# xyzy/jubatus

Measured on AMD Instinct MI355X. Metric: train_samples_per_sec, higher is better.
Workload: dtype fp32

## Files before the change

jubatus_amd/csrc/hip/jb_vc_state.hpp:

```cpp
#pragma once
#include <stdint.h>

#include "jb_serial_layout.hpp"

namespace jb {
namespace vc {

enum : int { kNew = 0, kRetry = 1, kDone = 2, kDense = 3 };
enum : int {
  S_MAGIC = 0, S_BEG, S_BEND, S_STATUS, S_LW, S_T, S_NCAND, S_PEND, S_WHY, S_NUPD, S_NSLOTS, S_VIOL,
  S_DONEB, S_NVALID, S_RETRYW, S_WEND,
  S_WINDOWS, S_RETRIES, S_STEPS, S_ROUNDS, S_WASTED, S_REFRESH, S_EXACT, S_CAND, S_UPD, S_SAT, S_TICKS,
  S_NONC, S_PH0, S_PH1, S_PH2, S_PH3, S_PH4, S_PHW, S_WIDE, S_DENSE_PM,
  S_DCHUNK,
  S_STEPPED,
  S_NCHUNK,
  S_BBEG,
  S_CSMODE,
  S_CSN,
  S_NWORDS = 64
};
enum : int { kWhyEnd = 0, kWhySat = 1, kWhyDense = 2 };
constexpr int64_t kDenseChunk0 = 8192, kDenseChunkMax = 1 << 20;

constexpr int kSpSlotBytes = 98304;
__host__ __device__ constexpr int sp_nslot(int lc) {
  return kSpSlotBytes / (8 * lc) > 1024 ? 1024 : kSpSlotBytes / (8 * lc);
}
__device__ __forceinline__ void sp_buckets(int row, int nb, int* b1, int* b2) {
  const uint32_t h1 = (uint32_t)row * 0x9E3779B1u;
  uint32_t h2 = ((uint32_t)row ^ 0x5bd1e995u) * 0x85EBCA77u;
  h2 ^= h2 >> 13;
  h2 *= 0xC2B2AE35u;
  *b1 = (int)__umulhi(h1, (uint32_t)nb);
  int c = (int)__umulhi(h2, (uint32_t)nb);
  if (c == *b1) c = c + 1 == nb ? 0 : c + 1;
  *b2 = c;
}
__device__ __forceinline__ int sp_find(const int32_t* key, int nb, int32_t row) {
  if (row < 0) return -1;
  int b1, b2;
  sp_buckets(row, nb, &b1, &b2);
  const int4 k1 = reinterpret_cast<const int4*>(key)[b1];
  const int4 k2 = reinterpret_cast<const int4*>(key)[b2];
  int s = -1;
  s = k1.x == row ? 4 * b1 : s;
  s = k1.y == row ? 4 * b1 + 1 : s;
  s = k1.z == row ? 4 * b1 + 2 : s;
  s = k1.w == row ? 4 * b1 + 3 : s;
  s = k2.x == row ? 4 * b2 : s;
  s = k2.y == row ? 4 * b2 + 1 : s;
  s = k2.z == row ? 4 * b2 + 2 : s;
  s = k2.w == row ? 4 * b2 + 3 : s;
  return s;
}

__device__ inline int64_t seg_estimate(const int64_t* st) {
  const int64_t wins = st[S_WINDOWS], stepped = st[S_STEPPED];
  const int64_t committed = st[S_BEG] - st[S_BBEG] - stepped;
  int64_t per = committed > 0 && wins > 0 ? committed / wins : 2048;
  per = per < 1024 ? 1024 : per;
  return wins + st[S_RETRIES] + (stepped + per - 1) / per;
}

}
}
```

jubatus_amd/csrc/hip/serial.hip:

```cpp
#include "jb_linear.hpp"
#include "jb_serial_layout.hpp"
#include <cstdio>
#include <cstdlib>
#include <algorithm>
#include <mutex>
#include <unordered_map>

namespace jb {

constexpr int kCommitThreads = 512;
constexpr int kDBits = 14;
constexpr int kDCap = 1 << kDBits;
constexpr int kDProbe = 32;
constexpr int kDFull = kDCap * 5 / 8;
constexpr int kBloomBits = 16;
constexpr int kSerialNF = 16;
constexpr float kSlackGuard = 1e-4f;
constexpr int kStepBits = 8;
constexpr int kStepCap = 1 << kStepBits;
constexpr int kStepList = 64;
constexpr int kSerialSegments = 4;
constexpr int kSerialSegmentsBig = 48;
constexpr int64_t kSerialBigBatch = 16384;
constexpr int kVerifiedSegmentsMin = 8;
constexpr int kVerifiedSegmentsMax = 2048;
constexpr int kRescoreWaste = 16;
constexpr int kScoreMaxBlocks = 8192;
#ifndef JB_SERIAL_TIMING
#define JB_SERIAL_TIMING 0
#endif
constexpr bool kSerialTiming = JB_SERIAL_TIMING != 0;
__device__ __forceinline__ uint64_t stamp() { return kSerialTiming ? clock64() : 0; }

template <int LC>
__device__ __forceinline__ void sample_scores_ro(const int32_t* __restrict__ fidx,
                                                 const float* __restrict__ fval, int64_t beg, int n,
                                                 const float* __restrict__ W, int lane,
                                                 float (&acc)[Lanes<LC>::K]) {
  using L = Lanes<LC>;
  const int g = lane / L::LW;
  const int l0 = lane % L::LW;
#pragma unroll
  for (int k = 0; k < L::K; ++k) acc[k] = 0.f;
  for (int j = g; j < n; j += L::G) {
    const int32_t idx = fidx[beg + j];
    const float x = fval[beg + j];
    if (idx >= 0) {
      const float* wr = W + (int64_t)idx * LC + l0;
#pragma unroll
      for (int k = 0; k < L::K; ++k) acc[k] += x * wr[64 * k];
    }
  }
#pragma unroll
  for (int off = L::LW; off < 64; off <<= 1) {
#pragma unroll
    for (int k = 0; k < L::K; ++k) acc[k] += __shfl_xor(acc[k], off, 64);
  }
}

template <int LC>
__device__ __forceinline__ float margin_of(const float (&acc)[Lanes<LC>::K], int y,
                                           const bool (&act)[Lanes<LC>::K], int lane, int* lstar,
                                           float* sy_out, float* best_out) {
  using L = Lanes<LC>;
  const int l0 = lane % L::LW;
  float sy = 0.f, best = -INFINITY;
  int bl = -1;
#pragma unroll
  for (int k = 0; k < L::K; ++k) {
    const int l = l0 + 64 * k;
    if (l == y) sy = acc[k];
    if (act[k] && l != y && acc[k] > best) { best = acc[k]; bl = l; }
  }
  sy = __shfl(sy, y % L::LW, 64);
  argmax_wrong<L::LW>(best, bl);
  *lstar = bl;
  *sy_out = sy;
  *best_out = bl >= 0 ? best : 0.f;
  return sy - (bl >= 0 ? best : 0.f);
}

__device__ __forceinline__ float decision_slack(int method, float margin, float nrm, bool has_l,
                                                float C, float sy, float best) {
  float s;
// ... 493 lines not shown
      if (k == INT_MAX) break;
      if (tid == k) {
        if (!loaded) load_features<NF>(fi, fx, live, nf, fb, fidx, fval);
        s_n = nf;
        s_y = yl;
        s_fb = fb;
        if (nf <= NF)
          for (int u = 0; u < nf; ++u) { s_fi[u] = fi[u]; s_fx[u] = fx[u]; }
      }
      if (wv == 0) {
        d.step_clear(lane);
        __builtin_amdgcn_wave_barrier();
        if (lane == 0) s_sn = 0;
      }
      lds_barrier();
      { const uint64_t t = stamp(); ph[2] += t - tc; tc = t; }
      if (wv == 0) {
        asm volatile("s_waitcnt vmcnt(0)" ::: "memory");
        const int n = s_n;
        bool up;
        if (kStaged && n <= NF)
          up = commit_staged<(LC <= 32 ? LC : 32)>(s_fi, s_fx, n, s_y, W, P, act[0], lane, method, C,
                                                   touched, d);
        else
          up = commit_sample<LC>(fidx, fval, s_fb, n, s_y, W, P, act, lane, method, C, touched, d);
        if (up) ++n_upd; else ++n_waste;
        if (lane == 0) s_waste = n_waste;
      }
      lim = k;
      ++steps;
      ++n_steps;
      { const uint64_t t = stamp(); ph[3] += t - tc; tc = t; }
      lds_barrier();
      { const uint64_t t = stamp(); ph[4] += t - tc; tc = t; }
      tw = stamp();
      if (s_sat || steps > bail_after || (rescore_waste > 0 && s_waste > rescore_waste)) {
        stop = p + k + 1;
        why = s_sat ? kStopSaturated : steps > bail_after ? kStopDense : kStopRescore;
        break;
      }
      if (loaded && open && tid > k && sl >= 0.f) {
        if (s_sn > kStepList || nf > NF) {
          bnd = full_bound();
        } else {
          bnd += d.step_bound<NF>(fi, fx);
        }
      }
    }
    ++n_rounds;
    const bool counted = live && !(sl != sl) && j < stop;
    const uint64_t cm = __builtin_amdgcn_ballot_w64(counted);
    if (lane == 0 && cm != 0) atomicAdd(&s_valid, (unsigned)__popcll(cm));
    if (stop != end) break;
  }
  __syncthreads();
  auto put = [&](int i, int64_t v) { tail[i] = seg == 0 ? v : tail[i] + v; };
  if (lane == 0) put(kTailBoundWave0 + wv, (int64_t)wwork);
  if (tid == 0) {
    tail[kTailStart] = stop;
    tail[kTailEnd] = end;
    tail[kTailReason] = why;
    put(kTailSteps, n_steps);
    put(kTailRounds, n_rounds);
    put(kTailSegments, 1);
    for (int i = 0; i < 6; ++i) put(kTailBoundPhase0 + i, (int64_t)ph[i]);
    put(kTailBoundWall, kSerialTiming ? (int64_t)(wall_clock64() - w0) : 0);
    put(kTailBoundCycles,
        (int64_t)(stamp() - tc) + (int64_t)(ph[0] + ph[1] + ph[2] + ph[3] + ph[4] + ph[5]));
    if (stats != nullptr && s_valid > 0) atomicAdd(stats + 1, (unsigned long long)s_valid);
  }
  if (tid == 0 && stats != nullptr && n_upd > 0) atomicAdd(stats, (unsigned long long)n_upd);
}

}

extern "C" int64_t jb_serial_scratch_bytes(int64_t n_max) {
  return jb::VcScratch::bytes(n_max > 0 ? n_max : 1);
}

extern "C" int64_t jb_serial_scratch_bytes_lc(int64_t n_max, int LC) {
  return LC > 64 ? jb::BoundScratch::bytes(n_max > 0 ? n_max : 1) : jb_serial_scratch_bytes(n_max);
}

enum : int { kSeenReason = 0, kSeenSegments, kSeenSegEst, kSeenWords };
static_assert(jb::kTailSegments == jb::kTailReason + 1, "one copy reads back both");
static std::mutex& seen_mu() {
  static std::mutex mu;
  return mu;
}
static std::unordered_map<void*, int64_t*>& seen_map() {
  static std::unordered_map<void*, int64_t*> seen;
  return seen;
}
static int64_t* segments_seen(void* scratch) {
  std::lock_guard<std::mutex> g(seen_mu());
  auto& seen = seen_map();
  auto it = seen.find(scratch);
  if (it != seen.end()) return it->second;
  int64_t* p = nullptr;
  if (hipHostMalloc((void**)&p, kSeenWords * sizeof(int64_t), hipHostMallocDefault) != hipSuccess) return nullptr;
  p[kSeenReason] = jb::kStopDone;
  p[kSeenSegments] = 128;
  p[kSeenSegEst] = 0;
  seen[scratch] = p;
  return p;
}

extern "C" int jb_vcommit_prepare(const int64_t* row_ptr, const int32_t* fidx, const float* fval,
                                  const int32_t* labels, const int64_t* stream_ptr, int nstreams, int64_t n_max,
                                  float* W, float* S, const int32_t* active, int LC, int method, float C,
                                  unsigned long long* stats, uint8_t* touched, void* scratch, int nseg,
                                  hipStream_t stream);

extern "C" int jb_serial_scratch_forget(void* scratch) {
  std::lock_guard<std::mutex> g(seen_mu());
  auto& seen = seen_map();
  auto it = seen.find(scratch);
  if (it == seen.end()) return 0;
  (void)hipHostFree(it->second);
  seen.erase(it);
  return 1;
}

static int segment_budget(int64_t n_max, int64_t prev, int64_t est, int64_t why) {
  if (n_max < jb::kSerialBigBatch) return jb::kVerifiedSegmentsMin;
  if (why != jb::kStopDone && why != jb::kStopDense) return jb::kVerifiedSegmentsMax;
  static const std::pair<int, int> slack = [] {
    const char* e = getenv("JB_VC_SEG_SLACK");
    int d = 2, c = 8;
    if (e != nullptr && sscanf(e, "%d,%d", &d, &c) != 2) { d = 2; c = 8; }
    return std::make_pair(d > 0 ? d : 2, c >= 0 ? c : 8);
  }();
  prev = std::max(prev, est);
  return (int)std::min<int64_t>(jb::kVerifiedSegmentsMax,
                                std::max<int64_t>(jb::kVerifiedSegmentsMin,
                                                  prev + prev / slack.first + slack.second));
}

extern "C" int jb_serial_prepare(const int64_t* row_ptr, const int32_t* fidx, const float* fval,
                                 const int32_t* labels, const int64_t* stream_ptr, int nstreams,
                                 int64_t n_max, float* W, float* S, const int32_t* active, int LC,
                                 int method, float C, unsigned long long* stats, uint8_t* touched,
                                 void* scratch, int64_t scratch_bytes, int bail_after,
                                 hipStream_t stream) {
  if (nstreams <= 0 || n_max <= 0) return 0;
  if (scratch == nullptr || scratch_bytes < jb_serial_scratch_bytes_lc(n_max, LC)) return -3;
  if (method >= jb::CW && S == nullptr) return -4;
  int64_t* tail = (int64_t*)scratch;
  if (LC <= 64) {
    volatile int64_t* seen = segments_seen(scratch);
    const int nseg = seen != nullptr
                         ? segment_budget(n_max, seen[kSeenSegments], seen[kSeenSegEst], seen[kSeenReason])
                         : segment_budget(n_max, 0, 0, jb::kStopDone);
    const int rc = jb_vcommit_prepare(row_ptr, fidx, fval, labels, stream_ptr, nstreams, n_max, W, S, active,
                                      LC, method, C, stats, touched, scratch, nseg, stream);
    if (rc == 0 && seen != nullptr) {
      int64_t* host = const_cast<int64_t*>(seen);
      (void)hipMemcpyAsync(host + kSeenReason, tail + jb::kTailReason, 2 * sizeof(int64_t), hipMemcpyDeviceToHost,
                           stream);
      (void)hipMemcpyAsync(host + kSeenSegEst, tail + jb::kTailSegEst, sizeof(int64_t), hipMemcpyDeviceToHost,
                           stream);
    }
    return rc;
  }
  float* slack = (float*)((uint8_t*)scratch + jb::BoundScratch::slack_offset());
  float* l1n = (float*)((uint8_t*)scratch + jb::BoundScratch::l1_offset(n_max));
  const int64_t blocks = std::min<int64_t>((n_max * 64 + 255) / 256, jb::kScoreMaxBlocks);
  const int nseg = n_max >= jb::kSerialBigBatch ? jb::kSerialSegmentsBig : jb::kSerialSegments;
  static_assert(jb::kTailStart == 0 && jb::kTailEnd == 1, "the tail doubles as a one-stream stream_ptr");
  for (int seg = 0; seg < nseg; ++seg) {
    const int waste = seg + 1 < nseg ? jb::kRescoreWaste : 0;
    const int64_t* sp = seg == 0 ? stream_ptr : tail;
    const int ns = seg == 0 ? nstreams : 1;
    const int64_t* why = seg == 0 ? nullptr : tail + jb::kTailReason;
#define JB_SERIAL(L)                                                                              \
  hipLaunchKernelGGL((jb::serial_score_kernel<L>), dim3((unsigned)blocks), dim3(256), 0, stream,  \
                     row_ptr, fidx, fval, labels, sp, ns, W, active, method, C, slack, l1n, why); \
  hipLaunchKernelGGL((jb::serial_commit_kernel<L>), dim3(1), dim3(jb::kCommitThreads), 0, stream, \
                     row_ptr, fidx, fval, labels, sp, ns, W, S, active, method, C, slack, l1n,    \
                     stats, touched, tail, bail_after, seg, waste);                               \
  break;
    switch (LC) {
      case 128: JB_SERIAL(128)
      case 256: JB_SERIAL(256)
      case 512: JB_SERIAL(512)
      case 1024: JB_SERIAL(1024)
      default: return -1;
    }
#undef JB_SERIAL
  }
  return (int)hipGetLastError();
}
```

jubatus_amd/csrc/hip/vcommit.hip:

```cpp
#include <string.h>

#include <type_traits>

#include "jb_commit.hpp"
#include "jb_vc_state.hpp"

namespace jb {
namespace vc {

using dc::Geo;
constexpr int kFCMax = 2;
constexpr int kRec = 16 * kFCMax;
constexpr int64_t kLwMin = 2048, kLwMax = kVcWindowMax, kLwInit = 8192;
constexpr int kBitWords = kVcBitWords;
constexpr float kTInit = 0.5f, kTMin = 0.125f, kTMax = 64.f;
constexpr int64_t kMagic = 0x56434f4d4d495433LL;
constexpr int kRetryForce = 3;

__device__ __forceinline__ float st_T(const int64_t* st) { return __int_as_float((int)st[S_T]); }
__device__ __forceinline__ int64_t ld_st(const int64_t* p) {
  return __hip_atomic_load(p, __ATOMIC_RELAXED, __HIP_MEMORY_SCOPE_AGENT);
}
__device__ __forceinline__ bool live(int status) { return status == kNew || status == kRetry; }

__device__ __forceinline__ float frcp(float x) { return __builtin_amdgcn_rcpf(x); }
__device__ __forceinline__ bool step_coeffs_fast(int method, float margin, float var, float nrm, bool has_l, float C,
                                                 float* tau, float* beta) {
  switch (method) {
    case PERCEPTRON:
      if (margin <= 0.f) { *tau = 1.f; *beta = 0.f; return true; }
      return false;
    case PA: case PA1: case PA2: {
      const float loss = 1.f - margin;
      if (!(loss > 0.f && nrm > 0.f)) return false;
      const float sq = (has_l ? 2.f : 1.f) * nrm;
      if (method == PA) *tau = loss * frcp(sq);
      else if (method == PA1) *tau = fminf(C, loss * frcp(sq));
      else *tau = loss * frcp(sq + 0.5f * frcp(C));
      *beta = 0.f;
      return true;
    }
    case CW: {
      if (!(var > 0.f)) return false;
      const float phi = C;
      const float b = 1.f + 2.f * phi * margin;
      const float disc = b * b - 8.f * phi * (margin - phi * var);
      const float gamma = (-b + sqrtf(fmaxf(disc, 0.f))) * frcp(4.f * phi * var);
      if (!(gamma > 0.f)) return false;
      *tau = gamma; *beta = 2.f * gamma * phi;
      return true;
    }
    case AROW:
      if (!(margin < 1.f)) return false;
      *beta = frcp(var + frcp(C));
      *tau = (1.f - margin) * *beta;
      return true;
    case NHERD: {
      if (!(margin < 1.f)) return false;
      *tau = (1.f - margin) * frcp(var + frcp(C));
      const float cv = 1.f + C * var;
      *beta = (C * C * var + 2.f * C) * frcp(cv * cv);
      return true;
    }
    default: return false;
  }
}
__device__ __forceinline__ float dprec_fast(int method, float beta, float x, float s) {
  const float bx2 = beta * x * x;
  return method == CW ? bx2 : bx2 * frcp(1.f - bx2 * s);
}

__global__ __launch_bounds__(256) void vc_init_kernel(int64_t* __restrict__ st, const int64_t* __restrict__ sp,
                                                      int nstreams, unsigned long long* __restrict__ bits,
                                                      int64_t* __restrict__ tail, float t_force,
                                                      int32_t* __restrict__ g_key, float* __restrict__ g_rmax,
                                                      int dense_pm) {
  for (int i = threadIdx.x; i < kBitWords; i += blockDim.x) bits[i] = 0ull;
  const bool fresh = st[S_MAGIC] != kMagic;
  if (fresh)
    for (int i = threadIdx.x; i < 1024; i += blockDim.x) { g_key[i] = -1; g_rmax[i] = 0.f; }
  __syncthreads();
  if (threadIdx.x != 0) return;
  if (fresh) {
    for (int i = 0; i < S_NWORDS; ++i) st[i] = 0;
    st[S_MAGIC] = kMagic;
    st[S_LW] = kLwInit;
    st[S_T] = __float_as_int(kTInit);
  }
  if (t_force > 0.f) st[S_T] = __float_as_int(t_force);
  const int64_t beg = sp[0], bend = sp[nstreams];
  st[S_BEG] = beg;
  st[S_BEND] = bend;
  st[S_WEND] = beg;
  st[S_STATUS] = beg < bend ? kNew : kDone;
  for (int i = S_NCAND; i <= S_RETRYW; ++i) st[i] = 0;
  for (int i = S_WINDOWS; i < S_NWORDS; ++i) st[i] = 0;
  st[S_DENSE_PM] = dense_pm;
  st[S_DCHUNK] = kDenseChunk0;
  st[S_BBEG] = beg;
  for (int i = 0; i < kTailWords; ++i) tail[i] = 0;
  tail[kTailStart] = beg < bend ? beg : bend;
  tail[kTailEnd] = bend;
  tail[kTailVerified] = 1;
}

// ... 136 lines not shown
  const int g = lane / L::LW;
  const int l0 = lane % L::LW;
  const bool la = l0 < LC && active[l0] != 0;
  for (int64_t k = ((int64_t)blockIdx.x * blockDim.x + tid) >> 6; k < ncand; k += nwaves) {
    int lo = 0, hi = nw - 1;
    while (lo < hi) {
      const int mid = (lo + hi + 1) >> 1;
      if (s_pref[mid] <= k) lo = mid; else hi = mid - 1;
    }
    unsigned long long word = bits[lo];
    for (int j = (int)k - s_pref[lo]; j > 0; --j) word &= word - 1;
    const int pos = 64 * lo + (__ffsll((long long)word) - 1);
    const int64_t s = beg + pos;
    int n;
    float acc, q;
    wave_score<LC>(row_ptr, fidx, fval, W, s, lane, la, &n, &acc, &q);
    const int64_t fb = row_ptr[s];
    if (lane < kRec) {
      const bool in = lane < n;
      FI[k * kRec + lane] = in ? fidx[fb + lane] : -1;
      FX[k * kRec + lane] = in ? fval[fb + lane] : 0.f;
    }
    if (lane == 0 && n > 16) atomicOr((unsigned long long*)&st[S_WIDE], 1ull);
    if (lane < LC) S0[k * LC + lane] = acc;
    (void)g;
    const int y = labels[s];
    if (y < 0 || y >= LC) {
      if (lane == 0) AUX[k] = make_int4(dc::aux_pack(-1, -1, n), __float_as_int(q), __float_as_int(1.f), pos);
      continue;
    }
    int bl;
    const float sl0 = wave_slack<LC>(acc, y, la, lane, method, C, q, &bl);
    if (lane == 0) AUX[k] = make_int4(dc::aux_pack(y, bl, n), __float_as_int(q), __float_as_int(sl0), pos);
    if (P == nullptr) continue;
    if (lane < kRec) {
      float2 pp = make_float2(1.f, 1.f);
      if (lane < n) {
        const int32_t idx = fidx[fb + lane];
        if (idx >= 0) {
          pp.x = P[(int64_t)idx * LC + y];
          if (bl >= 0) pp.y = P[(int64_t)idx * LC + bl];
        }
      }
      PP0[k * kRec + lane] = pp;
    }
  }
}

template <int LC, int FC>
struct Raw {
  int32_t fi[FC];
  float fx[FC];
  float2 pp[FC];
  float s[Geo<LC>::K];
  int aux;
  float nrm;
  float slack0;
  int pos;
};

template <int LC, int FC>
struct Samp {
  int32_t fi[FC];
  float fx[FC];
  float py[FC];
  float pl[FC];
  float s[Geo<LC>::K];
  int y;
  int ls0;
  int nf;
  float nrm;
  float slack0;
  int pos;
};

struct __attribute__((aligned(16))) Stamp { float sid, dy, dl, rmax; };

template <int LC, int MT, int R_, int PD_, int FC_>
__global__ __launch_bounds__(64) void vc_commit_kernel(
    int64_t* __restrict__ st, const float* __restrict__ W, const float* __restrict__ P,
    const int32_t* __restrict__ active, float C, const float* __restrict__ S0_k,
    const int4* __restrict__ AUX_k, const float2* __restrict__ PP0_k, const int32_t* __restrict__ FI_k,
    const float* __restrict__ FX_k, int32_t* __restrict__ g_key, float* __restrict__ g_rmax,
    float* __restrict__ g_dw, float* __restrict__ g_dp, int prof) {
  using Gm = Geo<LC>;
  using Rw = Raw<LC, FC_>;
  using S = Samp<LC, FC_>;
  constexpr int kFC = FC_;
  constexpr int kNFM = 16 * FC_;
  constexpr int kR = R_;
  constexpr int kNS = 4 * R_;
  constexpr int kPD = PD_;
  constexpr int K = Gm::K;
  constexpr int NSLOT = Gm::NSLOT;
  constexpr int method = MT;
  constexpr bool use_s = MT >= CW;
  constexpr bool use_nrm = MT == PA || MT == PA1 || MT == PA2 || MT == CW;
  constexpr float kG = dc::kGuard;
  if (!live((int)st[S_STATUS])) return;
  if (st[S_CSMODE] == 1) return;
  if ((st[S_WIDE] != 0) != (FC_ == 2)) return;
  __shared__ __attribute__((aligned(16))) float s_dw[NSLOT * LC + Gm::PAD];
  __shared__ __attribute__((aligned(16))) float s_dp[use_s ? NSLOT * LC + Gm::PAD : 4];
  __shared__ __attribute__((aligned(16))) int32_t s_key[NSLOT];
  __shared__ __attribute__((aligned(16))) Stamp s_sg[NSLOT + 1];

  const int lane = threadIdx.x;
  const int sub = lane & 15;
  const int G = lane >> 4;
  const uint64_t t_k0 = __builtin_amdgcn_s_memrealtime();
  const uint64_t t_c0 = __builtin_amdgcn_s_memtime();
  {
    float4* dw4 = reinterpret_cast<float4*>(s_dw);
    float4* dp4 = reinterpret_cast<float4*>(s_dp);
    const float4 z = make_float4(0.f, 0.f, 0.f, 0.f);
    for (int i = lane; i < (NSLOT * LC + Gm::PAD) / 4; i += 64) {
      dw4[i] = z;
      if (use_s) dp4[i] = z;
    }
    for (int i = lane; i < NSLOT; i += 64) s_key[i] = -1;
    for (int i = lane; i <= NSLOT; i += 64) s_sg[i] = Stamp{__int_as_float(-1), 0.f, 0.f, 0.f};
  }
  int act[K];
#pragma unroll
  for (int k = 0; k < K; ++k) {
    const int lab = sub + 16 * k;
    act[k] = (lab < LC && active[lab] != 0) ? 1 : 0;
  }
  const int64_t ncand = (int64_t)dc::in_vgpr((uint64_t)st[S_NCAND]);
  const int64_t wb = (int64_t)dc::in_vgpr((uint64_t)st[S_BEG]);
  const int64_t we = (int64_t)dc::in_vgpr((uint64_t)st[S_WEND]);
  const float* __restrict__ S0 = dc::in_vgpr(S0_k);
  const int4* __restrict__ AUX = dc::in_vgpr(AUX_k);
  const float2* __restrict__ PP0 = dc::in_vgpr(PP0_k);
  const int32_t* __restrict__ FI = dc::in_vgpr(FI_k);
  const float* __restrict__ FX = dc::in_vgpr(FX_k);

  auto load_raw = [&](int64_t k0, Rw (&rw)[kR]) {
#pragma unroll
    for (int r = 0; r < kR; ++r) {
      int64_t j = k0 + G * kR + r;
      j = j < ncand ? j : ncand - 1;
      j = j < 0 ? 0 : j;
#pragma unroll
      for (int c = 0; c < kFC; ++c) {
        const int64_t o = j * kRec + c * 16 + sub;
        rw[r].fi[c] = dc::gld(FI + o);
        rw[r].fx[c] = dc::gld(FX + o);
        if (use_s) rw[r].pp[c] = dc::gld(PP0 + o);
      }
#pragma unroll
      for (int k = 0; k < K; ++k) {
        const int lab = sub + 16 * k;
        rw[r].s[k] = dc::gld(S0 + j * LC + (lab < LC ? lab : LC - 1));
      }
      const int* a = reinterpret_cast<const int*>(AUX + j);
      rw[r].aux = dc::gld(a);
      rw[r].slack0 = __int_as_float(dc::gld(a + 2));
      rw[r].pos = dc::gld(a + 3);
      if (use_nrm) rw[r].nrm = __int_as_float(dc::gld(a + 1));
    }
  };
  auto unpack = [&](int64_t k0, const Rw (&rw)[kR], S (&sm)[kR]) {
#pragma unroll
    for (int r = 0; r < kR; ++r) {
      const bool ok = k0 + G * kR + r < ncand;
#pragma unroll
      for (int c = 0; c < kFC; ++c) {
        sm[r].fi[c] = ok ? rw[r].fi[c] : -1;
        sm[r].fx[c] = ok ? rw[r].fx[c] : 0.f;
        sm[r].py[c] = (use_s && ok) ? rw[r].pp[c].x : 1.f;
        sm[r].pl[c] = (use_s && ok) ? rw[r].pp[c].y : 1.f;
      }
#pragma unroll
      for (int k = 0; k < K; ++k) sm[r].s[k] = (ok && sub + 16 * k < LC) ? rw[r].s[k] : 0.f;
      const int aux = rw[r].aux;
      sm[r].y = ok ? dc::aux_y(aux) : -1;
      sm[r].ls0 = (use_s && ok) ? dc::aux_ls(aux) : -1;
      sm[r].nf = ok ? dc::aux_nf(aux) : 0;
      sm[r].nrm = (use_nrm && ok) ? rw[r].nrm : 0.f;
      sm[r].slack0 = ok ? rw[r].slack0 : 1.f;
      sm[r].pos = rw[r].pos;
    }
  };
// ... 270 lines not shown
            cy = row16_sum(cy);
            cl = row16_sum(cl);
            if (exact[r]) {
#pragma unroll
              for (int kk = 0; kk < K; ++kk) {
                const int lab = sub + 16 * kk;
                if (lab == yk) sc[r].s[kk] += cy;
                if (lab == lk) sc[r].s[kk] += cl;
              }
            }
            slack[r] -= (fabsf(cy) + fabsf(cl)) * (1.f + 4.f * kG);
            if (exact[r] && !(slack[r] > 0.f)) {
              int ls2;
              float sy2, best2;
              const float m2 = dc::group_margin<LC>(sc[r].s, sc[r].y, act, sub, &ls2, &sy2, &best2);
              slack[r] = dc::slack_of(method, m2, sc[r].nrm, ls2 >= 0, C, sy2, best2);
            }
          }
          make_exact(k);
#pragma unroll
          for (int r = 0; r < kR; ++r)
            if (G * kR + r > k) unsafe[r] = (alive[r] && (sc[r].nf > kNFM || !(slack[r] > 0.f))) ? 1 : 0;
        }
        return 0;
      };
      int stop_code = 0;
      switch (rk) {
        case 0: stop_code = step_of(std::integral_constant<int, 0>{}); break;
        case 1: if constexpr (kR > 1) stop_code = step_of(std::integral_constant<int, (kR > 1 ? 1 : 0)>{}); break;
        case 2: if constexpr (kR > 2) stop_code = step_of(std::integral_constant<int, (kR > 2 ? 2 : 0)>{}); break;
        default: if constexpr (kR > 3) stop_code = step_of(std::integral_constant<int, (kR > 3 ? 3 : 0)>{}); break;
      }
      stamp(4);
      if (stop_code) break;
      lim = k;
    }
    bump(3);
  };
  for (int64_t p0 = 0; p0 < ncand && !stopped; p0 += kPD * kNS) {
#pragma unroll
    for (int u = 0; u < kPD; ++u) {
      const int64_t p = p0 + u * kNS;
      unpack(p, pf[u], sc);
      load_raw(p + kPD * kNS, pf[u]);
      if (p < ncand && !stopped) round(p);
    }
  }
  int nslots = 0;
  for (int i = lane; i < NSLOT; i += 64) {
    const int32_t key = s_key[i];
    g_key[i] = key;
    g_rmax[i] = s_sg[i].rmax;
    nslots += key >= 0;
  }
  {
    constexpr int Q = LC / 4;
    for (int i = lane; i < NSLOT * Q; i += 64) {
      if (s_key[i / Q] < 0) continue;
      reinterpret_cast<float4*>(g_dw)[i] = reinterpret_cast<const float4*>(s_dw)[i];
      if (use_s) reinterpret_cast<float4*>(g_dp)[i] = reinterpret_cast<const float4*>(s_dp)[i];
    }
  }
#pragma unroll
  for (int off = 1; off < 64; off <<= 1) nslots += __shfl_xor(nslots, off, 64);
  if (lane == 0) {
    st[S_PEND] = pend;
    st[S_WHY] = why;
    st[S_NUPD] = s_cnt[0];
    st[S_NSLOTS] = nslots;
    st[S_STEPS] += n_steps;
    st[S_ROUNDS] += s_cnt[3];
    st[S_WASTED] += s_cnt[1];
    st[S_REFRESH] += s_cnt[2];
    st[S_EXACT] += n_exact;
    st[S_CAND] += ncand;
    st[S_TICKS] += (int64_t)(__builtin_amdgcn_s_memrealtime() - t_k0);
    if (kProf) {
      for (int i = 0; i < 5; ++i) st[S_PH0 + i] += (int64_t)s_ph[i];
      st[S_PHW] += (int64_t)(__builtin_amdgcn_s_memtime() - t_c0);
    }
  }
}

template <int LC>
__global__ __launch_bounds__(256) void vc_verify_kernel(
    int64_t* __restrict__ st, const int64_t* __restrict__ row_ptr, const int32_t* __restrict__ fidx,
    const float* __restrict__ fval, const int32_t* __restrict__ labels, const float* __restrict__ SL,
    unsigned long long* __restrict__ bits, const int32_t* __restrict__ g_key,
    const float* __restrict__ g_rmax, const float* __restrict__ g_dw, const float* __restrict__ g_dp,
    float* __restrict__ W, float* __restrict__ P, uint8_t* __restrict__ touched,
    unsigned long long* __restrict__ stats, int64_t* __restrict__ tail) {
  using Gm = Geo<LC>;
  constexpr int NSLOT = Gm::NSLOT;
  constexpr float kG = dc::kGuard;
  const int status = (int)st[S_STATUS];
  if (!live(status)) return;
  __shared__ __attribute__((aligned(16))) int32_t s_key[NSLOT];
  __shared__ float s_rmax[NSLOT];
  __shared__ unsigned s_valid, s_viol;
  __shared__ int s_last, s_force;
  const int tid = threadIdx.x;
  for (int i = tid; i < NSLOT; i += blockDim.x) {
    s_key[i] = g_key[i];
    s_rmax[i] = g_rmax[i];
  }
  if (tid == 0) { s_valid = 0; s_viol = 0; }
  __syncthreads();
  const int64_t wb = st[S_BEG], pe = st[S_PEND];
  const bool cs_mode = st[S_CSMODE] == 1;
  unsigned nvalid = 0, nviol = 0, nnonc = 0;
  for (int64_t i = wb + (int64_t)blockIdx.x * blockDim.x + tid; i < pe; i += (int64_t)gridDim.x * blockDim.x) {
    const int y = labels[i];
    if (y < 0 || y >= LC) continue;
    ++nvalid;
    const int64_t rel = i - wb;
    const unsigned long long bit = 1ull << (rel & 63);
    if (bits[rel >> 6] & bit) continue;
    ++nnonc;
    float bound = 0.f;
    for (int64_t j = row_ptr[i]; j < row_ptr[i + 1]; ++j) {
      const int32_t row = fidx[j];
      if (row < 0) continue;
      const int s = cs_mode ? sp_find(s_key, sp_nslot(LC) / 4, row) : dc::cache_find<LC>(s_key, row);
      if (s >= 0) bound += fabsf(fval[j]) * s_rmax[s];
    }
    bound *= 2.f * (1.f + 4.f * kG);
    if (!(SL[rel] > bound)) {
      atomicOr(bits + (rel >> 6), bit);
      ++nviol;
    }
  }
  if (nvalid) atomicAdd(&s_valid, nvalid);
  if (nviol) atomicAdd(&s_viol, nviol);
  if (nnonc) atomicAdd((unsigned long long*)&st[S_NONC], (unsigned long long)nnonc);
  __syncthreads();
  if (tid == 0) {
    if (s_valid) atomicAdd((unsigned long long*)&st[S_NVALID], (unsigned long long)s_valid);
    if (s_viol) atomicAdd((unsigned long long*)&st[S_VIOL], (unsigned long long)s_viol);
    __threadfence();
    s_last = atomicAdd((unsigned long long*)&st[S_DONEB], 1ull) == (unsigned long long)(gridDim.x - 1);
  }
  __syncthreads();
  if (!s_last) return;
  __threadfence();
  const int64_t viol = ld_st(&st[S_VIOL]);
  const int64_t wend = st[S_WEND];
  if (viol == 0) {
    __shared__ int s_used[NSLOT];
    __shared__ int s_nused;
    if (tid == 0) s_nused = 0;
    __syncthreads();
    for (int i = tid; i < NSLOT; i += blockDim.x)
      if (s_key[i] >= 0) s_used[atomicAdd(&s_nused, 1)] = i;
    __syncthreads();
    constexpr int Q = LC / 4;
    constexpr int kU = 4;
    const int items = s_nused * Q;
    for (int b0 = 0; b0 < items; b0 += kU * (int)blockDim.x) {
      float4 w[kU], d[kU], pv[kU], dp[kU];
      int64_t off[kU];
      bool on[kU];
#pragma unroll
      for (int u = 0; u < kU; ++u) {
        const int it = b0 + u * (int)blockDim.x + tid;
        on[u] = it < items;
        const int sl = s_used[on[u] ? it / Q : 0];
        const int q = it % Q;
        off[u] = (int64_t)s_key[sl] * Q + q;
        const int gi = sl * Q + q;
        if (on[u]) {
          w[u] = reinterpret_cast<const float4*>(W)[off[u]];
          d[u] = reinterpret_cast<const float4*>(g_dw)[gi];
          if (P != nullptr) {
            pv[u] = reinterpret_cast<const float4*>(P)[off[u]];
            dp[u] = reinterpret_cast<const float4*>(g_dp)[gi];
          }
        }
      }
#pragma unroll
      for (int u = 0; u < kU; ++u) {
        if (!on[u]) continue;
        w[u].x += d[u].x; w[u].y += d[u].y; w[u].z += d[u].z; w[u].w += d[u].w;
        reinterpret_cast<float4*>(W)[off[u]] = w[u];
        if (P != nullptr) {
          pv[u].x += dp[u].x; pv[u].y += dp[u].y; pv[u].z += dp[u].z; pv[u].w += dp[u].w;
          reinterpret_cast<float4*>(P)[off[u]] = pv[u];
        }
        if (off[u] % Q == 0 && touched != nullptr) touched[off[u] / Q] = 1;
      }
    }
    for (int i = tid; i < kBitWords; i += blockDim.x) bits[i] = 0ull;
    if (tid == 0) {
      const int64_t nupd = st[S_NUPD];
      const int64_t nv = ld_st(&st[S_NVALID]);
      if (stats != nullptr) {
        if (nupd > 0) atomicAdd(stats, (unsigned long long)nupd);
        if (nv > 0) atomicAdd(stats + 1, (unsigned long long)nv);
      }
      const int why = (int)st[S_WHY];
      const int64_t bend = st[S_BEND];
      st[S_BEG] = pe;
      st[S_WINDOWS] += 1;
      st[S_UPD] += nupd;
      if (why == kWhySat) st[S_SAT] += 1;
      const int64_t dpm = st[S_DENSE_PM];
      const bool dense = dpm > 0 && pe < bend && nupd * 1000 > dpm * (pe - wb);
      st[S_STATUS] = (why == kWhyDense || dense) ? kDense : (pe >= bend ? kDone : kNew);
      if (!(why == kWhyDense || dense)) st[S_DCHUNK] = kDenseChunk0;
      int64_t lw = st[S_LW];
      if (why == kWhySat) {
        const int64_t took = pe - wb;
        lw = took + took / 4;
      } else if (pe - wb >= lw) {
        lw = 2 * lw;
      }
      lw = lw < kLwMin ? kLwMin : (lw > kLwMax ? kLwMax : lw);
      st[S_LW] = lw;
      const float T = fmaxf(kTMin, st_T(st) * 0.97f);
      st[S_T] = __float_as_int(T);
      st[S_RETRYW] = 0;
    }
  } else {
    if (tid == 0) {
      st[S_RETRIES] += 1;
      st[S_RETRYW] += 1;
      const float T = fminf(kTMax, st_T(st) * 1.5f);
      st[S_T] = __float_as_int(T);
      st[S_STATUS] = kRetry;
      s_force = st[S_RETRYW] >= kRetryForce;
    }
    __syncthreads();
    if (s_force) {
      const int64_t n = wend - wb;
      for (int64_t w = tid; w < (n + 63) / 64; w += blockDim.x) {
        const int64_t rem = n - 64 * w;
        bits[w] = rem >= 64 ? ~0ull : ((1ull << rem) - 1);
      }
    }
  }
  __syncthreads();
  if (tid == 0) {
    st[S_DONEB] = 0;
    st[S_NVALID] = 0;
    st[S_VIOL] = 0;
    const int s2 = (int)st[S_STATUS];
    if (s2 != kRetry) st[S_WIDE] = 0;
    tail[kTailStart] = s2 == kDone ? st[S_BEND] : st[S_BEG];
    tail[kTailEnd] = st[S_BEND];
    tail[kTailSteps] = st[S_STEPS];
    tail[kTailRounds] = st[S_ROUNDS];
    tail[kTailReason] = s2 == kDone ? kStopDone : s2 == kDense ? kStopDense : kStopSaturated;
    tail[kTailSegments] = st[S_WINDOWS] + st[S_RETRIES];
    tail[kTailStepped] = st[S_STEPPED];
    tail[kTailChunks] = st[S_NCHUNK];
    tail[kTailSegEst] = seg_estimate(st);
    tail[kTailCsWindows] = st[S_CSN];
    tail[kTailWasted] = st[S_WASTED];
    tail[kTailRefresh] = st[S_REFRESH];
    tail[kTailUpdates] = st[S_UPD];
    tail[kTailRows] = st[S_NSLOTS];
    tail[kTailExact] = st[S_EXACT];
    tail[kTailCand] = st[S_CAND];
    tail[kTailRetries] = st[S_RETRIES];
    tail[kTailSatWindows] = st[S_SAT];
    tail[kTailTicks] = st[S_TICKS];
    for (int i = 0; i < 5; ++i) tail[kTailVcPhase0 + i] = st[S_PH0 + i];
    tail[kTailVcPhaseWall] = st[S_PHW];
    tail[kTailVcWindowLen] = st[S_LW];
    tail[kTailVcT] = st[S_T];
    tail[kTailVcNonCand] = st[S_NONC];
  }
}

}
}

extern "C" int64_t jb_vcommit_fixed_bytes() { return jb::kVcFixed; }

extern "C" int jb_stepper_enabled();
extern "C" int jb_stepper_chunk(const int64_t* row_ptr, const int32_t* fidx, const float* fval, const int32_t* labels,
                                float* W, float* P, const int32_t* active, int LC, int method, float C,
                                unsigned long long* stats, uint8_t* touched, int64_t* vst, int64_t* vtail,
                                hipStream_t stream);
extern "C" int jb_stepper_cand(const int64_t* row_ptr, const int32_t* fidx, const float* fval,
                               const int32_t* labels, float* W, float* P, const int32_t* active, int LC, int method,
                               float C, int64_t* vst, const int4* aux, int32_t* g_key, float* g_rmax, float* g_dw,
                               float* g_dp, hipStream_t stream);

template <int L>
static int launch_vc(int method, const int64_t* row_ptr, const int32_t* fidx, const float* fval,
                     const int32_t* labels, float* W, float* S, const int32_t* active, float C, int64_t* st,
                     float* sl, unsigned long long* bits, float* s0, int4* aux, float2* pp0, int32_t* fi,
                     float* fx, int32_t* gk, float* gr, float* gdw, float* gdp, uint8_t* touched,
                     unsigned long long* stats, int64_t* tail, int nseg, bool chunks, int cs_min, int cs_pm,
                     hipStream_t stream) {
  using namespace jb::vc;
  static const int prof = [] {
    const char* e = getenv("JB_COMMIT_PROF");
    return (e != nullptr && e[0] == '1') ? 1 : 0;
  }();
  static const bool r1pd1 = [] {
    const char* e = getenv("JB_VC_SHAPE");
    return e != nullptr && strcmp(e, "r1pd1") == 0;
  }();
  float* Pp = method >= jb::CW ? S : nullptr;
  for (int seg = 0; seg < nseg; ++seg) {
    hipLaunchKernelGGL((vc_score_kernel<L>), dim3(1024), dim3(256), 0, stream, st, row_ptr, fidx, fval, labels,
                       W, active, method, C, sl, bits, gk, gr);
    hipLaunchKernelGGL((vc_gather_kernel<L>), dim3(512), dim3(256), 0, stream, st, row_ptr, fidx, fval, labels,
                       W, Pp, active, method, C, bits, s0, aux, pp0, fi, fx, cs_min, cs_pm);
#define JB_VC_S(M, R, PD)                                                                                       \
  hipLaunchKernelGGL((vc_commit_kernel<L, M, R, PD, 1>), dim3(1), dim3(64), 0, stream, st, W, Pp, active, C, s0, \
                     aux, pp0, fi, fx, gk, gr, gdw, gdp, prof);                                                  \
  hipLaunchKernelGGL((vc_commit_kernel<L, M, R, PD, 2>), dim3(1), dim3(64), 0, stream, st, W, Pp, active, C, s0, \
                     aux, pp0, fi, fx, gk, gr, gdw, gdp, prof);
#define JB_VC_M(M)                               \
  if (r1pd1) { JB_VC_S(M, 1, 1) }                \
  else { JB_VC_S(M, 1, 2) }                      \
  break;
    switch (method) {
      case jb::PERCEPTRON: JB_VC_M(jb::PERCEPTRON)
      case jb::PA: JB_VC_M(jb::PA)
      case jb::PA1: JB_VC_M(jb::PA1)
      case jb::PA2: JB_VC_M(jb::PA2)
      case jb::CW: JB_VC_M(jb::CW)
      case jb::AROW: JB_VC_M(jb::AROW)
      case jb::NHERD: JB_VC_M(jb::NHERD)
      default: return -1;
    }
#undef JB_VC_M
#undef JB_VC_S
    if (cs_min > 0) {
      const int rc = jb_stepper_cand(row_ptr, fidx, fval, labels, W, Pp, active, L, method, C, st, aux, gk, gr, gdw,
                                     gdp, stream);
      if (rc != 0) return rc;
    }
    hipLaunchKernelGGL((vc_verify_kernel<L>), dim3(256), dim3(256), 0, stream, st, row_ptr, fidx, fval, labels,
                       sl, bits, gk, gr, gdw, gdp, W, Pp, touched, stats, tail);
    if (chunks) {
      const int rc = jb_stepper_chunk(row_ptr, fidx, fval, labels, W, Pp, active, L, method, C, stats, touched, st,
                                      tail, stream);
      if (rc != 0) return rc;
    }
  }
  return 0;
}

extern "C" int jb_vcommit_prepare(const int64_t* row_ptr, const int32_t* fidx, const float* fval,
                                  const int32_t* labels, const int64_t* stream_ptr, int nstreams, int64_t n_max,
                                  float* W, float* S, const int32_t* active, int LC, int method, float C,
                                  unsigned long long* stats, uint8_t* touched, void* scratch, int nseg,
                                  hipStream_t stream) {
  if (LC > 64) return -1;
  using Lay = jb::VcScratch;
  int64_t* tail = (int64_t*)scratch;
  uint8_t* base = (uint8_t*)scratch;
  float* s0 = (float*)(base + Lay::offset(Lay::S0, n_max));
  float2* pp0 = (float2*)(base + Lay::offset(Lay::PP0, n_max));
  int32_t* fi = (int32_t*)(base + Lay::offset(Lay::FI, n_max));
  float* fx = (float*)(base + Lay::offset(Lay::FX, n_max));
  int4* aux = (int4*)(base + Lay::offset(Lay::AUX, n_max));
  float* sl = (float*)(base + Lay::offset(Lay::SL, n_max));
  uint8_t* fixed = base + Lay::fixed_offset(n_max);
  int64_t* st = (int64_t*)fixed;
  unsigned long long* bits = (unsigned long long*)(fixed + jb::kVcStateBytes);
  int32_t* gk = (int32_t*)(bits + jb::kVcBitWords);
  float* gr = (float*)(gk + jb::kVcStoreRows);
  float* gdw = gr + jb::kVcStoreRows;
  float* gdp = gdw + jb::kVcStoreFloats;
  const char* te = getenv("JB_VERIFIED_T");
  const float t_force = te != nullptr ? (float)atof(te) : 0.f;
  const char* de = getenv("JB_VC_DENSE_PM");
  const int dense_pm = de != nullptr ? atoi(de) : 300;
  hipLaunchKernelGGL(jb::vc::vc_init_kernel, dim3(1), dim3(256), 0, stream, st, stream_ptr, nstreams, bits, tail,
                     t_force, gk, gr, dense_pm);
  const bool chunks = dense_pm > 0 && jb_stepper_enabled();
  const char* cs_e = getenv("JB_VC_CS");
  const char* cs_p = getenv("JB_VC_CS_PM");
  const int cs_min = (jb_stepper_enabled() && cs_e != nullptr) ? atoi(cs_e) : 0;
  const int cs_pm = cs_p != nullptr ? atoi(cs_p) : 350;
  int rc = 0;
#define JB_VC_L(L)                                                                                            \
  rc = launch_vc<L>(method, row_ptr, fidx, fval, labels, W, S, active, C, st, sl, bits, s0, aux, pp0, fi, fx, \
                    gk, gr, gdw, gdp, touched, stats, tail, nseg, chunks, cs_min, cs_pm, stream);              \
  break;
  switch (LC) {
    case 8: JB_VC_L(8)
    case 16: JB_VC_L(16)
    case 32: JB_VC_L(32)
    case 64: JB_VC_L(64)
    default: return -1;
  }
#undef JB_VC_L
  if (rc) return rc;
  return (int)hipGetLastError();
}
```

Before: 262.6 million.

## Adaptively skip wide commit and chunk launches; widen verify kernel and pack counters

The host now reads back more tail words (stepped, chunks, reason, segment estimate, wide-window count) after each call. It uses them to skip launching the FC=2 wide commit kernel when no wide windows occurred, and to run the dense stepper chunk only every fourth segment when the previous call needed none. The verify kernel moves to 512 threads with 16 lanes per row and packs the valid, nonc and viol counts plus the block-done count into one 64-bit atomic. The segment budget slack heuristic is also retuned. The aim is fewer kernel launches and atomics per segment, at the cost of relying on history from the previous call, which may mispredict when the input changes.

```diff
diff --git a/jubatus_amd/csrc/hip/jb_vc_state.hpp b/jubatus_amd/csrc/hip/jb_vc_state.hpp
--- a/jubatus_amd/csrc/hip/jb_vc_state.hpp
+++ b/jubatus_amd/csrc/hip/jb_vc_state.hpp
@@ -18,6 +18,7 @@
   S_BBEG,
   S_CSMODE,
   S_CSN,
+  S_WIDEB,
   S_NWORDS = 64
 };
 enum : int { kWhyEnd = 0, kWhySat = 1, kWhyDense = 2 };
diff --git a/jubatus_amd/csrc/hip/serial.hip b/jubatus_amd/csrc/hip/serial.hip
--- a/jubatus_amd/csrc/hip/serial.hip
+++ b/jubatus_amd/csrc/hip/serial.hip
@@ -1,5 +1,6 @@
 #include "jb_linear.hpp"
 #include "jb_serial_layout.hpp"
+#include "jb_vc_state.hpp"
 #include <cstdio>
 #include <cstdlib>
 #include <algorithm>
@@ -659,8 +660,12 @@
   return LC > 64 ? jb::BoundScratch::bytes(n_max > 0 ? n_max : 1) : jb_serial_scratch_bytes(n_max);
 }
 
-enum : int { kSeenReason = 0, kSeenSegments, kSeenSegEst, kSeenWords };
-static_assert(jb::kTailSegments == jb::kTailReason + 1, "one copy reads back both");
+enum : int { kSeenStepped = 0, kSeenChunks, kSeenSegEst, kSeenCsWindows, kSeenReason, kSeenSegments, kSeenWide,
+             kSeenWords };
+static_assert(jb::kTailChunks == jb::kTailStepped + kSeenChunks && jb::kTailSegEst == jb::kTailStepped + kSeenSegEst &&
+                  jb::kTailReason == jb::kTailStepped + kSeenReason &&
+                  jb::kTailSegments == jb::kTailStepped + kSeenSegments,
+              "one copy reads back the tail words");
 static std::mutex& seen_mu() {
   static std::mutex mu;
   return mu;
@@ -676,9 +681,11 @@
   if (it != seen.end()) return it->second;
   int64_t* p = nullptr;
   if (hipHostMalloc((void**)&p, kSeenWords * sizeof(int64_t), hipHostMallocDefault) != hipSuccess) return nullptr;
+  for (int i = 0; i < kSeenWords; ++i) p[i] = 0;
   p[kSeenReason] = jb::kStopDone;
   p[kSeenSegments] = 128;
-  p[kSeenSegEst] = 0;
+  p[kSeenChunks] = 1;
+  p[kSeenWide] = 1;
   seen[scratch] = p;
   return p;
 }
@@ -687,7 +694,7 @@
                                   const int32_t* labels, const int64_t* stream_ptr, int nstreams, int64_t n_max,
                                   float* W, float* S, const int32_t* active, int LC, int method, float C,
                                   unsigned long long* stats, uint8_t* touched, void* scratch, int nseg,
-                                  hipStream_t stream);
+                                  int wide, int chunk_every, hipStream_t stream);
 
 extern "C" int jb_serial_scratch_forget(void* scratch) {
   std::lock_guard<std::mutex> g(seen_mu());
@@ -704,14 +711,15 @@
   if (why != jb::kStopDone && why != jb::kStopDense) return jb::kVerifiedSegmentsMax;
   static const std::pair<int, int> slack = [] {
     const char* e = getenv("JB_VC_SEG_SLACK");
-    int d = 2, c = 8;
-    if (e != nullptr && sscanf(e, "%d,%d", &d, &c) != 2) { d = 2; c = 8; }
-    return std::make_pair(d > 0 ? d : 2, c >= 0 ? c : 8);
+    int d = 4, c = 2;
+    if (e != nullptr && sscanf(e, "%d,%d", &d, &c) != 2) { d = 4; c = 2; }
+    return std::make_pair(d > 0 ? d : 4, c >= 0 ? c : 2);
   }();
+  const bool rough = est > prev;
   prev = std::max(prev, est);
+  const int64_t extra = rough ? prev / 2 + 8 : prev / slack.first + slack.second;
   return (int)std::min<int64_t>(jb::kVerifiedSegmentsMax,
-                                std::max<int64_t>(jb::kVerifiedSegmentsMin,
-                                                  prev + prev / slack.first + slack.second));
+                                std::max<int64_t>(jb::kVerifiedSegmentsMin, prev + extra));
 }
 
 extern "C" int jb_serial_prepare(const int64_t* row_ptr, const int32_t* fidx, const float* fval,
@@ -729,14 +737,19 @@
     const int nseg = seen != nullptr
                          ? segment_budget(n_max, seen[kSeenSegments], seen[kSeenSegEst], seen[kSeenReason])
                          : segment_budget(n_max, 0, 0, jb::kStopDone);
+    constexpr int kChunkEvery = 4;
+    const bool dense = seen == nullptr || seen[kSeenChunks] != 0 || seen[kSeenStepped] != 0 ||
+                       seen[kSeenReason] != jb::kStopDone;
+    const int wide = seen == nullptr || seen[kSeenWide] != 0;
     const int rc = jb_vcommit_prepare(row_ptr, fidx, fval, labels, stream_ptr, nstreams, n_max, W, S, active,
-                                      LC, method, C, stats, touched, scratch, nseg, stream);
+                                      LC, method, C, stats, touched, scratch, nseg, wide, dense ? 1 : kChunkEvery,
+                                      stream);
     if (rc == 0 && seen != nullptr) {
       int64_t* host = const_cast<int64_t*>(seen);
-      (void)hipMemcpyAsync(host + kSeenReason, tail + jb::kTailReason, 2 * sizeof(int64_t), hipMemcpyDeviceToHost,
-                           stream);
-      (void)hipMemcpyAsync(host + kSeenSegEst, tail + jb::kTailSegEst, sizeof(int64_t), hipMemcpyDeviceToHost,
-                           stream);
+      const int64_t* st = (const int64_t*)((const uint8_t*)scratch + jb::VcScratch::fixed_offset(n_max));
+      (void)hipMemcpyAsync(host + kSeenStepped, tail + jb::kTailStepped, (kSeenSegments + 1) * sizeof(int64_t),
+                           hipMemcpyDeviceToHost, stream);
+      (void)hipMemcpyAsync(host + kSeenWide, st + jb::vc::S_WIDEB, sizeof(int64_t), hipMemcpyDeviceToHost, stream);
     }
     return rc;
   }
diff --git a/jubatus_amd/csrc/hip/vcommit.hip b/jubatus_amd/csrc/hip/vcommit.hip
--- a/jubatus_amd/csrc/hip/vcommit.hip
+++ b/jubatus_amd/csrc/hip/vcommit.hip
@@ -18,9 +18,6 @@
 constexpr int kRetryForce = 3;
 
 __device__ __forceinline__ float st_T(const int64_t* st) { return __int_as_float((int)st[S_T]); }
-__device__ __forceinline__ int64_t ld_st(const int64_t* p) {
-  return __hip_atomic_load(p, __ATOMIC_RELAXED, __HIP_MEMORY_SCOPE_AGENT);
-}
 __device__ __forceinline__ bool live(int status) { return status == kNew || status == kRetry; }
 
 __device__ __forceinline__ float frcp(float x) { return __builtin_amdgcn_rcpf(x); }
@@ -323,7 +320,7 @@
     const int32_t* __restrict__ active, float C, const float* __restrict__ S0_k,
     const int4* __restrict__ AUX_k, const float2* __restrict__ PP0_k, const int32_t* __restrict__ FI_k,
     const float* __restrict__ FX_k, int32_t* __restrict__ g_key, float* __restrict__ g_rmax,
-    float* __restrict__ g_dw, float* __restrict__ g_dp, int prof) {
+    float* __restrict__ g_dw, float* __restrict__ g_dp, int prof, int solo) {
   using Gm = Geo<LC>;
   using Rw = Raw<LC, FC_>;
   using S = Samp<LC, FC_>;
@@ -340,7 +337,7 @@
   constexpr float kG = dc::kGuard;
   if (!live((int)st[S_STATUS])) return;
   if (st[S_CSMODE] == 1) return;
-  if ((st[S_WIDE] != 0) != (FC_ == 2)) return;
+  if (!solo && (st[S_WIDE] != 0) != (FC_ == 2)) return;
   __shared__ __attribute__((aligned(16))) float s_dw[NSLOT * LC + Gm::PAD];
   __shared__ __attribute__((aligned(16))) float s_dp[use_s ? NSLOT * LC + Gm::PAD : 4];
   __shared__ __attribute__((aligned(16))) int32_t s_key[NSLOT];
@@ -777,8 +774,9 @@
   }
 }
 
+constexpr int kVerifyThreads = 512, kVerifyBlocks = 256;
 template <int LC>
-__global__ __launch_bounds__(256) void vc_verify_kernel(
+__global__ __launch_bounds__(kVerifyThreads) void vc_verify_kernel(
     int64_t* __restrict__ st, const int64_t* __restrict__ row_ptr, const int32_t* __restrict__ fidx,
     const float* __restrict__ fval, const int32_t* __restrict__ labels, const float* __restrict__ SL,
     unsigned long long* __restrict__ bits, const int32_t* __restrict__ g_key,
@@ -792,53 +790,70 @@
   if (!live(status)) return;
   __shared__ __attribute__((aligned(16))) int32_t s_key[NSLOT];
   __shared__ float s_rmax[NSLOT];
-  __shared__ unsigned s_valid, s_viol;
+  __shared__ unsigned s_valid, s_viol, s_nonc;
+  __shared__ unsigned long long s_tot;
   __shared__ int s_last, s_force;
   const int tid = threadIdx.x;
   for (int i = tid; i < NSLOT; i += blockDim.x) {
     s_key[i] = g_key[i];
     s_rmax[i] = g_rmax[i];
   }
-  if (tid == 0) { s_valid = 0; s_viol = 0; }
+  if (tid == 0) { s_valid = 0; s_viol = 0; s_nonc = 0; }
   __syncthreads();
   const int64_t wb = st[S_BEG], pe = st[S_PEND];
   const bool cs_mode = st[S_CSMODE] == 1;
   unsigned nvalid = 0, nviol = 0, nnonc = 0;
-  for (int64_t i = wb + (int64_t)blockIdx.x * blockDim.x + tid; i < pe; i += (int64_t)gridDim.x * blockDim.x) {
+  const int sub = tid & 15;
+  const int64_t ngroups = (int64_t)gridDim.x * (blockDim.x >> 4);
+  for (int64_t i = wb + (int64_t)blockIdx.x * (blockDim.x >> 4) + (tid >> 4); i < pe; i += ngroups) {
+    const int64_t rel = i - wb;
     const int y = labels[i];
-    if (y < 0 || y >= LC) continue;
-    ++nvalid;
-    const int64_t rel = i - wb;
+    const unsigned long long word = bits[rel >> 6];
+    const int64_t fb = row_ptr[i], fe = row_ptr[i + 1];
+    const float sl = SL[rel];
+    const bool valid = y >= 0 && y < LC;
     const unsigned long long bit = 1ull << (rel & 63);
-    if (bits[rel >> 6] & bit) continue;
+    const bool nonc = valid && (word & bit) == 0;
+    float b = 0.f;
+    if (nonc) {
+      for (int64_t j = fb + sub; j < fe; j += 16) {
+        const int32_t row = fidx[j];
+        const int s = row < 0 ? -1
+                              : cs_mode ? sp_find(s_key, sp_nslot(LC) / 4, row) : dc::cache_find<LC>(s_key, row);
+        if (s >= 0) b += fabsf(fval[j]) * s_rmax[s];
+      }
+    }
+    const float bound = row16_sum(b) * (2.f * (1.f + 4.f * kG));
+    if (sub != 0) continue;
+    nvalid += valid;
+    if (!nonc) continue;
     ++nnonc;
-    float bound = 0.f;
-    for (int64_t j = row_ptr[i]; j < row_ptr[i + 1]; ++j) {
-      const int32_t row = fidx[j];
-      if (row < 0) continue;
-      const int s = cs_mode ? sp_find(s_key, sp_nslot(LC) / 4, row) : dc::cache_find<LC>(s_key, row);
-      if (s >= 0) bound += fabsf(fval[j]) * s_rmax[s];
-    }
-    bound *= 2.f * (1.f + 4.f * kG);
-    if (!(SL[rel] > bound)) {
+    if (!(sl > bound)) {
       atomicOr(bits + (rel >> 6), bit);
       ++nviol;
     }
   }
   if (nvalid) atomicAdd(&s_valid, nvalid);
   if (nviol) atomicAdd(&s_viol, nviol);
-  if (nnonc) atomicAdd((unsigned long long*)&st[S_NONC], (unsigned long long)nnonc);
+  if (nnonc) atomicAdd(&s_nonc, nnonc);
   __syncthreads();
+  constexpr int kCntBits = 17;
+  constexpr unsigned long long kCntMask = (1ull << kCntBits) - 1;
+  static_assert(kVcWindowMax <= (int64_t)kCntMask, "a window's counts fit their fields");
   if (tid == 0) {
-    if (s_valid) atomicAdd((unsigned long long*)&st[S_NVALID], (unsigned long long)s_valid);
-    if (s_viol) atomicAdd((unsigned long long*)&st[S_VIOL], (unsigned long long)s_viol);
+    const unsigned long long add = (unsigned long long)s_valid | ((unsigned long long)s_nonc << kCntBits) |
+                                   ((unsigned long long)s_viol << (2 * kCntBits)) | (1ull << (3 * kCntBits));
     __threadfence();
-    s_last = atomicAdd((unsigned long long*)&st[S_DONEB], 1ull) == (unsigned long long)(gridDim.x - 1);
+    const unsigned long long tot = atomicAdd((unsigned long long*)&st[S_DONEB], add) + add;
+    s_last = (tot >> (3 * kCntBits)) == (unsigned long long)gridDim.x;
+    s_tot = tot;
   }
   __syncthreads();
   if (!s_last) return;
   __threadfence();
-  const int64_t viol = ld_st(&st[S_VIOL]);
+  const int64_t n_valid = (int64_t)(s_tot & kCntMask);
+  const int64_t n_nonc = (int64_t)((s_tot >> kCntBits) & kCntMask);
+  const int64_t viol = (int64_t)((s_tot >> (2 * kCntBits)) & kCntMask);
   const int64_t wend = st[S_WEND];
   if (viol == 0) {
     __shared__ int s_used[NSLOT];
@@ -849,7 +864,7 @@
       if (s_key[i] >= 0) s_used[atomicAdd(&s_nused, 1)] = i;
     __syncthreads();
     constexpr int Q = LC / 4;
-    constexpr int kU = 4;
+    constexpr int kU = 8;
     const int items = s_nused * Q;
     for (int b0 = 0; b0 < items; b0 += kU * (int)blockDim.x) {
       float4 w[kU], d[kU], pv[kU], dp[kU];
@@ -887,7 +902,7 @@
     for (int i = tid; i < kBitWords; i += blockDim.x) bits[i] = 0ull;
     if (tid == 0) {
       const int64_t nupd = st[S_NUPD];
-      const int64_t nv = ld_st(&st[S_NVALID]);
+      const int64_t nv = n_valid;
       if (stats != nullptr) {
         if (nupd > 0) atomicAdd(stats, (unsigned long long)nupd);
         if (nv > 0) atomicAdd(stats + 1, (unsigned long long)nv);
@@ -936,10 +951,12 @@
   __syncthreads();
   if (tid == 0) {
     st[S_DONEB] = 0;
-    st[S_NVALID] = 0;
-    st[S_VIOL] = 0;
+    st[S_NONC] += n_nonc;
     const int s2 = (int)st[S_STATUS];
-    if (s2 != kRetry) st[S_WIDE] = 0;
+    if (s2 != kRetry) {
+      if (st[S_WIDE] != 0) st[S_WIDEB] += 1;
+      st[S_WIDE] = 0;
+    }
     tail[kTailStart] = s2 == kDone ? st[S_BEND] : st[S_BEG];
     tail[kTailEnd] = st[S_BEND];
     tail[kTailSteps] = st[S_STEPS];
@@ -987,8 +1004,8 @@
                      const int32_t* labels, float* W, float* S, const int32_t* active, float C, int64_t* st,
                      float* sl, unsigned long long* bits, float* s0, int4* aux, float2* pp0, int32_t* fi,
                      float* fx, int32_t* gk, float* gr, float* gdw, float* gdp, uint8_t* touched,
-                     unsigned long long* stats, int64_t* tail, int nseg, bool chunks, int cs_min, int cs_pm,
-                     hipStream_t stream) {
+                     unsigned long long* stats, int64_t* tail, int nseg, bool chunks, int chunk_every, bool wide,
+                     int cs_min, int cs_pm, hipStream_t stream) {
   using namespace jb::vc;
   static const int prof = [] {
     const char* e = getenv("JB_COMMIT_PROF");
@@ -1006,9 +1023,10 @@
                        W, Pp, active, method, C, bits, s0, aux, pp0, fi, fx, cs_min, cs_pm);
 #define JB_VC_S(M, R, PD)                                                                                       \
   hipLaunchKernelGGL((vc_commit_kernel<L, M, R, PD, 1>), dim3(1), dim3(64), 0, stream, st, W, Pp, active, C, s0, \
-                     aux, pp0, fi, fx, gk, gr, gdw, gdp, prof);                                                  \
-  hipLaunchKernelGGL((vc_commit_kernel<L, M, R, PD, 2>), dim3(1), dim3(64), 0, stream, st, W, Pp, active, C, s0, \
-                     aux, pp0, fi, fx, gk, gr, gdw, gdp, prof);
+                     aux, pp0, fi, fx, gk, gr, gdw, gdp, prof, wide ? 0 : 1);                                    \
+  if (wide)                                                                                                     \
+    hipLaunchKernelGGL((vc_commit_kernel<L, M, R, PD, 2>), dim3(1), dim3(64), 0, stream, st, W, Pp, active, C,   \
+                       s0, aux, pp0, fi, fx, gk, gr, gdw, gdp, prof, 0);
 #define JB_VC_M(M)                               \
   if (r1pd1) { JB_VC_S(M, 1, 1) }                \
   else { JB_VC_S(M, 1, 2) }                      \
@@ -1030,9 +1048,9 @@
                                      gdp, stream);
       if (rc != 0) return rc;
     }
-    hipLaunchKernelGGL((vc_verify_kernel<L>), dim3(256), dim3(256), 0, stream, st, row_ptr, fidx, fval, labels,
-                       sl, bits, gk, gr, gdw, gdp, W, Pp, touched, stats, tail);
-    if (chunks) {
+    hipLaunchKernelGGL((vc_verify_kernel<L>), dim3(kVerifyBlocks), dim3(kVerifyThreads), 0, stream, st, row_ptr,
+                       fidx, fval, labels, sl, bits, gk, gr, gdw, gdp, W, Pp, touched, stats, tail);
+    if (chunks && ((seg + 1) % chunk_every == 0 || seg + 1 == nseg)) {
       const int rc = jb_stepper_chunk(row_ptr, fidx, fval, labels, W, Pp, active, L, method, C, stats, touched, st,
                                       tail, stream);
       if (rc != 0) return rc;
@@ -1045,7 +1063,7 @@
                                   const int32_t* labels, const int64_t* stream_ptr, int nstreams, int64_t n_max,
                                   float* W, float* S, const int32_t* active, int LC, int method, float C,
                                   unsigned long long* stats, uint8_t* touched, void* scratch, int nseg,
-                                  hipStream_t stream) {
+                                  int wide, int chunk_every, hipStream_t stream) {
   if (LC > 64) return -1;
   using Lay = jb::VcScratch;
   int64_t* tail = (int64_t*)scratch;
@@ -1070,6 +1088,7 @@
   hipLaunchKernelGGL(jb::vc::vc_init_kernel, dim3(1), dim3(256), 0, stream, st, stream_ptr, nstreams, bits, tail,
                      t_force, gk, gr, dense_pm);
   const bool chunks = dense_pm > 0 && jb_stepper_enabled();
+  const bool both = wide != 0 || !chunks;
   const char* cs_e = getenv("JB_VC_CS");
   const char* cs_p = getenv("JB_VC_CS_PM");
   const int cs_min = (jb_stepper_enabled() && cs_e != nullptr) ? atoi(cs_e) : 0;
@@ -1077,7 +1096,8 @@
   int rc = 0;
 #define JB_VC_L(L)                                                                                            \
   rc = launch_vc<L>(method, row_ptr, fidx, fval, labels, W, S, active, C, st, sl, bits, s0, aux, pp0, fi, fx, \
-                    gk, gr, gdw, gdp, touched, stats, tail, nseg, chunks, cs_min, cs_pm, stream);              \
+                    gk, gr, gdw, gdp, touched, stats, tail, nseg, chunks, chunk_every > 0 ? chunk_every : 1,    \
+                    both, cs_min, cs_pm, stream);                                                             \
   break;
   switch (LC) {
     case 8: JB_VC_L(8)
```

Measured after the change: 260.0 million. Within noise of the previous version (-1.0%).
